# RoboticExplorationLab/TrajectoryOptimization.jl

Hardware: AMD Instinct MI355X
Metric: iLQR iterations/sec (batched trajectories) (higher is better)
Workload: dtype f64

## Files before the change

trajectoryoptimization.jl_amd/csrc/common.h:

```cpp
#pragma once
#include <hip/hip_runtime.h>

#include "models.h"
#include "problem_dev.h"

namespace to {

struct KArgs {
  DevProblem P;
  double* Xs;
  double* Us;
  double *Xc, *Uc;
  int dump_wave;
  int repack_block0;
  int CW, TW;
  double* x0;
  int* acc;
  int* accp;
  int coop_merge;
  int compact;
  int* alist;
  int* acount;
  int* ccount;
  double *Mc, *Hc, *gc;
  double* Kt;
  double *Mt, *Ht, *gt;
  int bwd_mfma;
  int bwd_lane;
  int h_compact;
  int h_diag;
  double *lam, *mu;
  double *J, *dJ, *grad, *rho, *drho, *dV, *cmax, *Jout;
  int *status, *iterations, *it_inner, *outer, *dJzero, *ls_index, *active, *budget, *bpfail;
  int* counter;
  int *oflag, *ost;
  int *olist, *ocount;
  double* knotbuf;
  double* mu_next;
  int* it_pn;
  double* pn_cmax;
  int al_mode;
  int control;
  int step;
  int ls_phase;
  int ls_c0;
  int blk0;
  int* pending;
  int* plist;
  int* pcount;
  int store_x;
};

struct PolicyArgs {
  int S;
  int TPW;
  int WPT;
  int g0;
  int store;
  int clamp;
  double alpha;
  double u_min[TO_MAX_M], u_max[TO_MAX_M];
  double mp[16];
  const double* x0s;
  double *J, *cmax, *dxmax;
  int *status, *klim;
  double *Xw, *Uw;
  const double* plants;
  double sigma_w[TO_MAX_N];
  double sigma_v[TO_MAX_N];
  unsigned long long seed;
  unsigned traj_offset, sample_offset;
};

template <class M> struct Gains { static constexpr int RSK = M::m * (M::ne + 1); };

#define TILE_PTR(base, L) ((base) + ((size_t)tile * (size_t)(L)) * 64 + lane)
#define EL(p, e) (p)[(size_t)(e) * 64]
#define TILE_LANE() const int tile = blockIdx.x, lane = threadIdx.x, b = tile * 64 + lane
__device__ __forceinline__ double* slot_ptr(double* nominal, double* cand, const int* accp, int b, int sl, int L) {
  if (sl == 0) return nominal + ((size_t)(b >> 6) * (size_t)L) * 64 + (b & 63);
  const int pos = accp[b];
  return cand + ((size_t)(pos >> 6) * (size_t)L) * 64 + (pos & 63);
}
#define X_SLOT_PTR(a, b, sl) slot_ptr((a).Xs, (a).Xc, (a).accp, b, sl, (a).P.N * (a).P.n)
#define U_SLOT_PTR(a, b, sl) slot_ptr((a).Us, (a).Uc, (a).accp, b, sl, ((a).P.N - 1) * (a).P.m)

template <class M, bool GEN = true, class D = std::nullptr_t>
__device__ __forceinline__ double knot_cost(const DevProblem& P, int k, const double* x, const double* u, const double* lam0,
                                            const double* mu0, bool with_al, const double* gl0 = nullptr, const double* cp0 = nullptr,
                                            const double* cl0 = nullptr, D dt0 = nullptr) {
  constexpr int n = M::n, m = M::m, nz = n + m;
  const int cidx = P.cost_index[k];
  double Jk = cost_eval<n, m, GEN>(P.costs[cidx], x, u);
  if constexpr (GEN) {
    if (P.gl) Jk += goal_lin_cost<n, m>(gl0, cidx, x, u);
  }
  if (P.opts.cost_dt_scaling && k < P.N - 1) Jk *= step_dt(P, k, dt0);
  if (with_al && P.n_cons > 0) {
    double z[nz];
#pragma unroll
    for (int i = 0; i < n; ++i) z[i] = x[i];
#pragma unroll
    for (int i = 0; i < m; ++i) z[n + i] = u[i];
// ... 157 lines not shown
```

trajectoryoptimization.jl_amd/csrc/handle.h:

```cpp
#pragma once
#include <hip/hip_runtime.h>

#include <atomic>
#include <condition_variable>
#include <cstdint>
#include <mutex>
#include <string>
#include <thread>
#include <type_traits>
#include <vector>

#include "common.h"
#include "path_plan.h"
#include "rp_plan.h"

namespace to {

int fail(int code, const std::string& msg);

#define HIPCHECK(expr)                                                                         \
  do {                                                                                         \
    hipError_t e_ = (expr);                                                                    \
    if (e_ != hipSuccess)                                                                      \
      return ::to::fail(TO_ERR_HIP, std::string(#expr) + ": " + hipGetErrorString(e_));        \
  } while (0)
#define TRY(expr) do { int r_ = (expr); if (r_ != TO_OK) return r_; } while (0)

constexpr int BLOCK = 64;

template <class... P, class... A>
inline void enqueue(void (*kernel)(P...), dim3 grid, dim3 block, size_t lds, hipStream_t stream, const A&... args) {
  hipLaunchKernelGGL(kernel, grid, block, lds, stream, args...);
}
inline int launched() {
  HIPCHECK(hipGetLastError());
  return TO_OK;
}
template <class... P, class... A>
inline int launch(void (*kernel)(P...), dim3 grid, dim3 block, size_t lds, hipStream_t stream, const A&... args) {
  enqueue(kernel, grid, block, lds, stream, args...);
  return launched();
}

struct ModelOps;

}

struct to_handle_s {
  int device = 0;
  hipStream_t stream = nullptr;
  int model_key = -1;
  const to::ModelOps* ops = nullptr;
  int R = 0, G = 0;
  to::KArgs a;
  std::vector<to_cost_desc> costs;
  std::vector<to::DevCon> cons;
  std::vector<double> dt;
  std::vector<int> cost_index;
  std::vector<double> step_table;
  std::vector<void*> allocs;
  double* stage = nullptr;
  size_t stage_bytes = 0;
  int* counter_host = nullptr;
  int counter_len = 0;
  to::PathTraits traits;
  to::PathPlan plan;
  int accept_chunks = 1;
  to_cost_desc* d_costs = nullptr;
  to::DevCon* d_cons = nullptr;
  double* d_dt = nullptr;
  int* d_cost_index = nullptr;
  int* d_crow = nullptr;
  std::vector<char> gl_set;
  double* d_gl = nullptr;
  double* d_pm = nullptr;
  std::vector<double> pm_host;
  bool pm_own = false;
  double* d_dtb = nullptr;
  std::vector<double> dtb_host;
  double* d_cp = nullptr;
  double* d_cl = nullptr;
  std::vector<int> cl_base;
  std::vector<std::vector<double>> cl_host;
  double* d_tmp = nullptr;
  double* d_tmp2 = nullptr;
  void* comm = nullptr;
  int comm_rank = 0, comm_size = 1;
  std::vector<int32_t> comm_counts;
  long long comm_offset = 0, comm_total = 0;
  bool comm_equal = true;
  double* pn_ws = nullptr;
  size_t pn_ws_bytes = 0;
  int* pn_pak = nullptr;
  long long* pn_koff = nullptr;
  int* pn_list = nullptr;
  int* pn_list_host = nullptr;
  int pn_tab_len = 0;
  int pn_cap = 0, pn_nbmax = 0;
  long long pn_per = 0;
  hipStream_t pn_stream = nullptr;
  hipEvent_t pn_ev[3] = {nullptr, nullptr, nullptr};
  int32_t *snap_status = nullptr, *snap_active = nullptr;
  double* snap_cmax = nullptr;
  int pn_early = 0;
  std::vector<char> pn_done_early;
  int pn_early_slots = 0;
  to_solver_opts pn_opts;
  double pn_early_ms = 0.0;
  struct RpArr { size_t off; int kind; int L; };
  std::vector<RpArr> rp_arr;
  std::vector<void*> rp_home, rp_work[2];
  int* rp_map[2] = {nullptr, nullptr};
  to::RpSized rp_sized[2];
  int rp_level = 0;
  int rp_B = 0, rp_Bp = 0;
  double *pol_x0s = nullptr, *pol_J = nullptr, *pol_cmax = nullptr, *pol_dxmax = nullptr;
  int *pol_status = nullptr, *pol_klim = nullptr;
  size_t pol_cap = 0;
  double *pol_xw = nullptr, *pol_uw = nullptr;
// ... 104 lines not shown
```

trajectoryoptimization.jl_amd/csrc/k_forward.h:

```cpp
#pragma once
#include <type_traits>

#include "common.h"
#include "ls_round.h"

#ifndef TO_FWD_WAVES
#define TO_FWD_WAVES 1
#endif
namespace to {

template <class M, bool WITHK>
struct FwdKnot {
  static constexpr int n = M::n, m = M::m, RSK = Gains<M>::RSK;
  double x[n], u[m], kd[WITHK ? RSK : 1];
  __device__ __forceinline__ void load(const double* pXk, const double* pUk, const double* pKk) {
#pragma unroll
    for (int i = 0; i < n; ++i) x[i] = EL(pXk, i);
#pragma unroll
    for (int j = 0; j < m; ++j) u[j] = EL(pUk, j);
    if constexpr (WITHK) {
#pragma unroll
      for (int i = 0; i < RSK; ++i) kd[i] = pKk[i];
    }
  }
};

template <class M>
__device__ __forceinline__ void stage_gains(const double* Kt, int b, int TW, int k, int N, double* kbuf, int hw) {
  constexpr int RSK = Gains<M>::RSK;
  static_assert(RSK % 2 == 0, "gains rows must be whole 16-byte pieces");
  constexpr int PCS = RSK / 2;
  typedef __attribute__((address_space(1))) const void* gptr_t;
  typedef __attribute__((address_space(3))) void* lptr_t;
  const int pieces = TW * PCS;
  for (int i0 = 0; i0 < pieces; i0 += 64) {
    const int gl = i0 + hw;
    int t = gl / PCS;
    const int off = gl - t * PCS;
    t = t < TW ? t : TW - 1;
    const int bt = __shfl(b, t);
    const char* src = (const char*)(Kt + ((size_t)bt * (N - 1) + k) * RSK) + off * 16;
    __builtin_amdgcn_global_load_lds((gptr_t)src, (lptr_t)((char*)kbuf + (size_t)i0 * 16), 16, 0, 0);
  }
}
template <class M>
__host__ __device__ inline int gains_lds_doubles(int TW) {
  constexpr int PCS = Gains<M>::RSK / 2;
  return ((TW * PCS + 63) / 64) * 64 * 2;
}

template <class M, int MODE>
__device__ __forceinline__ void forward_candidate(const KArgs& a, int tile, int lane, int b, bool live, double alpha, int wblock, double* kbuf,
                                                  int kbuf_len, int krow, int b0, int TW, int hw, double& J_out, double& g_out, bool& ok_out) {
  constexpr int n = M::n, m = M::m, ne = M::ne, RSK = Gains<M>::RSK;
  constexpr bool SIMPLE = (MODE & 1) != 0, CONS = (MODE & 2) != 0, GEN = (MODE & 8) != 0;
  constexpr bool KLDS = M::lds_gains;
// ... 634 lines not shown
        if (ncs > 0) Ja += cs0.term(ub);
        if (ncs > 1) Ja += cs1.term(ub);
        Jk += Ja;
      } else Jk += knot_al_cached<M, GEN>(P, k, xb, ub, lam0, mu0, ncs, cs0, cs1, cp0, cl0);
    }
    J += Jk;
    double mx = 0.0, mu_ = 0.0;
    if (k > 0) {
#pragma unroll
      for (int i = 0; i < n; ++i) { const double v = fabs(xb[i]); if (!(v <= mx)) mx = v; }
    }
#pragma unroll
    for (int j = 0; j < m; ++j) { const double v = fabs(ub[j]); if (!(v <= mu_)) mu_ = v; }
    if (!(mx <= max_x) || !(mu_ <= max_u)) ok = false;
  }
  FWD2_BARRIER();
  {
    double xb[n + 1];
    const double2* slot = (const double2*)(ring + (size_t)((N - 1) & 1) * R::SLOT) + hw;
#pragma unroll
    for (int pr = 0; pr < (n + 1) / 2; ++pr) { const double2 v = slot[pr * 64]; xb[2 * pr] = v.x; if (2 * pr + 1 < n + 1) xb[2 * pr + 1] = v.y; }
    double mx = 0.0;
#pragma unroll
    for (int i = 0; i < n; ++i) { const double v = fabs(xb[i]); if (!(v <= mx)) mx = v; }
    if (!(mx <= max_x)) ok = false;
#pragma unroll
    for (int i = 0; i < n; ++i) EL(pXo, i) = xb[i];
    double u0[m];
#pragma unroll
    for (int j = 0; j < m; ++j) u0[j] = 0.0;
    J += knot_cost<M, GEN>(P, N - 1, xb, u0, lam0, mu0, true, gl0, cp0, cl0);
  }
  J_out = J; g_out = gsum / (N - 1); ok_out = ok;
}

#ifndef TO_FWD2_WAVES
#define TO_FWD2_WAVES 1
#endif
template <class M>
__host__ __device__ inline size_t fwd2_lds_doubles(int TW) {
  return (M::lds_gains ? 2 * (size_t)gains_lds_doubles<M>(TW) + StageCostLds<M::n, M::m>::size : 0) + 2 * (size_t)Fwd2Ring<M>::SLOT + 2;
}
template <class M, int MODE>
__global__ void __launch_bounds__(128, TO_FWD2_WAVES) k_forward2(KArgs a) {
  extern __shared__ double kbuf[];
  const DevProblem& P = a.P;
  const to_solver_opts& o = P.opts;
  const int hw = threadIdx.x & 63;
  const int role = __builtin_amdgcn_readfirstlane(threadIdx.x >> 6);
  const int CW = a.CW, TW = a.TW;
  const int q = hw / TW, t = hw - q * TW;
  const int b0 = blockIdx.x * TW;
  int b, inrange;
  if (a.compact) {
    const int cnt = a.acount[a.step & 1];
    if (b0 >= cnt) return;
    inrange = (b0 + t) < cnt;
    b = a.alist[(size_t)(a.step & 1) * P.Bp + (inrange ? b0 + t : cnt - 1)];
  } else {
    inrange = (b0 + t) < P.B;
    b = (b0 + t) < P.Bp ? b0 + t : P.Bp - 1;
  }
  const int tile = b >> 6, lane = b & 63;
  const bool act = inrange && a.active[b] != 0;
  if (__ballot(act) == 0) return;
  const bool bpfail = act && a.bpfail[b] != 0;
  const int total = o.iterations_linesearch;
  const double Jprev = a.J[b];
  const double dV0 = a.dV[b], dV1 = a.dV[(size_t)P.Bp + b];
  const bool zero_step = act && !bpfail && (-(dV0 + dV1) <= 1e-12 * (1.0 + fabs(Jprev)));
  bool need = act && !bpfail && !zero_step;
  int accepted = zero_step ? 0 : -1, acc = 0, accpos = 0;
  double Jnew = Jprev, grad = 0.0;
  const double f = o.line_search_decrease_factor;
  const int kbuf_len = M::lds_gains ? gains_lds_doubles<M>(TW) : 0;
  const unsigned long long tmask = TW >= 64 ? ~0ull : (1ull << TW) - 1ull;
  double* ctab = kbuf + 2 * (size_t)kbuf_len;
  double* ring = ctab + (M::lds_gains ? StageCostLds<M::n, M::m>::size : 0);
  unsigned long long* needmask = (unsigned long long*)(ring + 2 * (size_t)Fwd2Ring<M>::SLOT);
  if constexpr (!LsRepack<M>::value) {
    const int krow = t * Gains<M>::RSK;
    unsigned long long nm = __ballot(need);
    for (int c0 = 0; c0 < total; c0 += CW) {
      if (nm == 0) break;
      const double alpha = ls_alpha(f, c0 + q, total);
      if (role == 0) {
        fwd2_roll<M, MODE>(a, tile, lane, b, alpha, kbuf, kbuf_len, krow, TW, hw, ring);
      } else {
        const bool cand = need && q < CW && (c0 + q) < total;
        double J, gm;
        bool ok;
        fwd2_account<M, MODE>(a, tile, lane, b, cand, (int)blockIdx.x, ctab, hw, ring, J, gm, ok);
        bool accept = false;
        if (cand && ok) {
          const double expected = -alpha * (dV0 + alpha * dV1);
          const double z = (expected > 0.0) ? (Jprev - J) / expected : -1.0;
          accept = z >= o.line_search_lower_bound && z <= o.line_search_upper_bound;
        }
        const unsigned long long am = __ballot(accept);
        int qs = -1;
        for (int qq = CW - 1; qq >= 0; --qq) qs = ((am >> (qq * TW + t)) & 1ull) ? qq : qs;
        const int src = (qs >= 0 ? qs : 0) * TW + t;
        const double Js = __shfl(J, src), gs = __shfl(gm, src);
        if (need && qs >= 0) { Jnew = Js; grad = gs; accepted = c0 + qs; acc = qs + 1; accpos = (int)blockIdx.x * 64 + src; need = false; }
        const unsigned long long left = __ballot(need);
        if (hw == 0) *needmask = left;
      }
// ... 53 lines not shown
```

trajectoryoptimization.jl_amd/csrc/k_misc.h:

```cpp
#pragma once
#include "common.h"

namespace to {

template <class M, int FIXED_INTEG, bool PM = false, bool DT = false>
__global__ void __launch_bounds__(64) k_rollout(KArgs a) {
  constexpr int n = M::n, m = M::m;
  TILE_LANE();
  const DevProblem& P = a.P;
  if (b >= P.B) return;
  constexpr int c = 0;
  double* X = X_SLOT_PTR(a, b, c);
  const double* U = U_SLOT_PTR(a, b, c);
  const double* x0 = TILE_PTR(a.x0, n);
  double x[n], u[m], xn[n];
  double pmr[PM ? 16 : 1];
  const double* mp = P.mp;
  if constexpr (PM) { load_plant(P, b, pmr); mp = pmr; }
  const double* dt0 = dt_lane_of<DT>(P, b);
#pragma unroll
  for (int i = 0; i < n; ++i) { x[i] = EL(x0, i); EL(X, i) = x[i]; }
  int lim = 0;
  const double max_x = P.opts.max_state_value, max_u = P.opts.max_control_value;
  for (int k = 0; k < P.N - 1; ++k) {
#pragma unroll
    for (int i = 0; i < m; ++i) u[i] = EL(U, k * m + i);
    model_step<M, double, FIXED_INTEG>(mp, P.integrator, k, x, u, step_dt_of<DT>(P, k, dt0), xn);
    double mx = 0.0, mu = 0.0;
#pragma unroll
    for (int i = 0; i < n; ++i) { x[i] = xn[i]; EL(X, (k + 1) * n + i) = x[i]; const double v = fabs(x[i]); mx = !(v <= mx) ? v : mx; }
#pragma unroll
    for (int i = 0; i < m; ++i) { const double v = fabs(u[i]); mu = !(v <= mu) ? v : mu; }
    if (lim == 0) lim = !(mx <= max_x) ? TO_STATE_LIMIT : !(mu <= max_u) ? TO_CONTROL_LIMIT : 0;
  }
  if (a.control && lim != 0 && a.active[b] != 0) {
    a.status[b] = lim; a.active[b] = 0;
    if (a.al_mode) a.outer[b] = 1;
  }
}

template <class M>
__global__ void __launch_bounds__(64) k_cost(KArgs a, int with_al, double* out, double* Jk) {
  constexpr int n = M::n, m = M::m;
  TILE_LANE();
  const DevProblem& P = a.P;
  if (b >= P.B) return;
  const int N = P.N;
  if (Jk) {
    constexpr int c = 0;
    const double* X = X_SLOT_PTR(a, b, c);
    const double* U = U_SLOT_PTR(a, b, c);
    double* o = TILE_PTR(Jk, N);
    const double* dt0 = dt_lane(P, b);
    for (int k = 0; k < N; ++k) {
      double x[n], u[m];
#pragma unroll
      for (int i = 0; i < n; ++i) x[i] = EL(X, k * n + i);
#pragma unroll
      for (int i = 0; i < m; ++i) u[i] = (k < N - 1) ? EL(U, k * m + i) : 0.0;
      EL(o, k) = knot_cost<M>(P, k, x, u, nullptr, nullptr, false, TILE_PTR(P.gl, P.n_costs * (n + m)), nullptr, nullptr, dt0);
    }
    return;
  }
  double J;
  trajectory_pass<M>(a, tile, lane, with_al != 0, false, &J, nullptr);
  out[b] = J;
}

template <class M>
__global__ void __launch_bounds__(64) k_violation(KArgs a, double* out) {
  TILE_LANE();
  if (b >= a.P.B) return;
  double cm;
  trajectory_pass<M>(a, tile, lane, false, false, nullptr, &cm);
  out[b] = cm;
}

template <class M>
__global__ void __launch_bounds__(64) k_dual_update(KArgs a) {
  TILE_LANE();
  const DevProblem& P = a.P;
  if (b >= P.B) return;
  trajectory_pass<M>(a, tile, lane, false, true, nullptr, nullptr);
  double* mu0 = TILE_PTR(a.mu, P.n_cons);
  for (int ci = 0; ci < P.n_cons; ++ci) EL(mu0, ci) = fmin(EL(mu0, ci) * P.opts.penalty_scaling, P.opts.penalty_max);
}


#define OUTER_LANE(FLAG)                                                                      \
  const DevProblem& P = a.P;                                                                  \
  const int cnt_ = a.ocount[a.step & 1];                                                      \
// ... 271 lines not shown
```

trajectoryoptimization.jl_amd/csrc/k_scan.h:

```cpp
#pragma once
#include "common.h"
#include "k_backward.h"
#include "k_expand.h"
#include "scan_combine.h"

namespace to {

__device__ __forceinline__ double scan_shfl(double v, int src_lane) {
  return __shfl(v, src_lane);
}

template <int n, bool VALUE_ONLY, bool SELECT>
__device__ __forceinline__ void scan_round(const ScanEl<n>& el, int l, int d, ScanEl<n>& out) {
  using E = ScanEl<n>;
  E pe;
  const int src = l + d;
  const bool has = src < 64;
  const int sl = has ? src : 63;
  if constexpr (VALUE_ONLY) {
#pragma unroll
    for (int i = 0; i < n; ++i) pe.eta[i] = scan_shfl(el.eta[i], sl);
#pragma unroll
    for (int i = 0; i < E::NSY; ++i) pe.J[i] = scan_shfl(el.J[i], sl);
    if constexpr (SELECT) {
      if (!has) {
#pragma unroll
        for (int i = 0; i < n; ++i) pe.eta[i] = 0.0;
#pragma unroll
        for (int i = 0; i < E::NSY; ++i) pe.J[i] = 0.0;
      }
    }
  } else {
    const double* pv = (const double*)&el;
    double* po = (double*)&pe;
#pragma unroll
    for (int i = 0; i < E::NV; ++i) po[i] = scan_shfl(pv[i], sl);
    if constexpr (SELECT) {
      if (!has) pe.identity();
    }
  }
  scan_combine<n, VALUE_ONLY>(el, pe, out);
}

template <class M>
__device__ __forceinline__ bool scan_element(const double* Mk, const double* Hd, const double* g, bool terminal, bool beyond,
                                             ScanEl<M::ne>& e) {
  constexpr int m = M::m, ne = M::ne, nc = ne + m;
  using E = ScanEl<ne>;
  bool ok = true;
  double iR[m];
#pragma unroll
  for (int c = 0; c < m; ++c) { if (!terminal && not_positive(Hd[ne + c])) ok = false; iR[c] = rcp_fast(terminal ? 1.0 : Hd[ne + c]); }
#pragma unroll
  for (int i = 0; i < ne; ++i) {
// ... 142 lines not shown
#pragma unroll
    for (int i = 0; i < ne; ++i) {
      double t = Qxx[i][j];
#pragma unroll
      for (int r = 0; r < m; ++r) t += Kg[r][i] * W[r][j];
#pragma unroll
      for (int r = 0; r < m; ++r) t += Qux[r][i] * Kg[r][j];
      Sn[i][j] = t;
    }
    double t = gq[j];
#pragma unroll
    for (int r = 0; r < m; ++r) t += Kg[r][j] * qd[r];
#pragma unroll
    for (int r = 0; r < m; ++r) t += Qux[r][j] * dk[r];
    sn[j] = t;
  }
  double dv1 = 0.0, dv2 = 0.0;
#pragma unroll
  for (int r = 0; r < m; ++r) {
    dv1 += dk[r] * gq[ne + r];
    double t = 0.0;
#pragma unroll
    for (int q = 0; q < m; ++q) t += Quu[r][q] * dk[q];
    dv2 += dk[r] * t;
  }
  dv1o = dv1; dv2o = 0.5 * dv2;
#pragma unroll
  for (int i = 0; i < ne; ++i) {
#pragma unroll
    for (int j = 0; j < ne; ++j) S[i][j] = 0.5 * (Sn[i][j] + Sn[j][i]);
    s[i] = sn[i];
  }
  return pd_ok;
}

#ifndef TO_SCAN_PRIO
#define TO_SCAN_PRIO 1
#endif
template <class M, int FIXED_INTEG, int VAR, bool TRIM = true>
__global__ void __launch_bounds__(64, 1) k_expand_backward_scan(KArgs a) {
  static_assert(!M::lie && M::ne <= 4 && M::m <= 2, "scan backward pass: small vector-space models");
  constexpr int n = M::n, m = M::m, ne = M::ne, nc = ne + m, RSK = Gains<M>::RSK;
  constexpr int PK = ne * nc + 2 * nc;
  using E = ScanEl<ne>;
  using LL = LaneLay<M>;
  __shared__ double park[2 * PK * 64];
#if TO_SCAN_PRIO
  if constexpr (TRIM) __builtin_amdgcn_s_setprio(TO_SCAN_PRIO);
#endif
  const DevProblem& P = a.P;
  const int N = P.N;
  const int b = blockIdx.x, l = threadIdx.x;
  const int tile = b >> 6, lane = b & 63;
  double rho = a.rho[b], drho = a.drho[b];
  if (!a.active[b]) return;
  const int c = M::accept_write_through ? a.acc[b] : 0;
  const double* X = X_SLOT_PTR(a, b, c);
  const double* U = U_SLOT_PTR(a, b, c);
  double* X0 = X_SLOT_PTR(a, b, 0);
  double* U0 = U_SLOT_PTR(a, b, 0);
  const bool wt = M::accept_write_through && c != 0;
  bool ok = true;
  E el;
  {
    E e0, e1;
#pragma unroll
    for (int kk = 0; kk < 2; ++kk) {
      const int kr = 2 * l + kk;
      const bool beyond = kr > N - 1;
      const int k = beyond ? N - 1 : kr;
      const bool terminal = (k == N - 1);
      double x[n], u[m];
#pragma unroll
      for (int i = 0; i < n; ++i) x[i] = EL(X, k * n + i);
#pragma unroll
      for (int i = 0; i < m; ++i) u[i] = terminal ? 0.0 : EL(U, k * m + i);
      if (wt && !beyond) {
#pragma unroll
        for (int i = 0; i < n; ++i) EL(X0, k * n + i) = x[i];
        if (!terminal) {
#pragma unroll
          for (int i = 0; i < m; ++i) EL(U0, k * m + i) = u[i];
        }
      }
      double Mk[ne * nc], H[LL::NS], g[nc], Hd[nc];
#pragma unroll
      for (int i = 0; i < ne * nc; ++i) Mk[i] = 0.0;
      expand_lane_knot<M, FIXED_INTEG, VAR>(a, tile, lane, k, x, u, Mk, H, g, a.P.mp);
#pragma unroll
      for (int j = 0; j < nc; ++j) { Hd[j] = (terminal && j >= ne) ? 1.0 : H[LL::sym(j, j)]; if (terminal && j >= ne) g[j] = 0.0; }
      double* pk = park + (size_t)kk * PK * 64 + l;
#pragma unroll
      for (int i = 0; i < ne * nc; ++i) pk[i * 64] = Mk[i];
#pragma unroll
      for (int j = 0; j < nc; ++j) { pk[(ne * nc + j) * 64] = Hd[j]; pk[(ne * nc + nc + j) * 64] = g[j]; }
      const bool eok = scan_element<M>(Mk, Hd, g, terminal, beyond, kk == 0 ? e0 : e1);
      if (!eok && !beyond) ok = false;
    }
    scan_combine<ne>(e0, e1, el);
  }
  double dV0 = 0.0, dV1 = 0.0;
  double* pK = a.Kt + ((size_t)b * (N - 1)) * RSK;
  bool done = false, failed = false;
  const bool elements_ok = __ballot(!ok) == 0;
  if (rho == 0.0 && elements_ok) {
    const int NB = (N + 1) / 2;
    int d = 1;
  #pragma unroll 1
    for (; (TRIM ? 2 * d : d) < NB; d <<= 1) {
      E out;
      scan_round<ne, false, !TRIM>(el, l, d, out);
      el = out;
    }
    if constexpr (TRIM) {
      if (d < NB) {
        E out;
        scan_round<ne, true, false>(el, l, d, out);
  #pragma unroll
        for (int i = 0; i < ne; ++i) el.eta[i] = out.eta[i];
  #pragma unroll
        for (int i = 0; i < E::NSY; ++i) el.J[i] = out.J[i];
      }
    }
    double S[ne][ne], s[ne];
    {
      const int src = (l + 1 < 64) ? l + 1 : 63;
      double Jn[E::NSY], en[ne];
  #pragma unroll
      for (int i = 0; i < E::NSY; ++i) Jn[i] = scan_shfl(el.J[i], src);
// ... 97 lines not shown
```

trajectoryoptimization.jl_amd/csrc/ops.h:

```cpp
#pragma once
#include <cstdlib>
#include <type_traits>

#include "handle.h"
#include "k_backward.h"
#include "k_expand.h"
#include "k_forward.h"
#include "k_scan.h"
#include "k_misc.h"
#include "k_policy.h"

namespace to {

template <class M>
void fill_traits(ModelOps& o) {
  o.write_through = M::accept_write_through;
  o.mfma_backward = M::mfma_backward;
  o.coop_backward = M::coop_backward;
  o.lane_backward = M::lane_backward;
  o.lds_gains = M::lds_gains;
  o.expand_knots = M::expand_knots;
  o.ls_first_round = M::ls_first_round;
  o.gains_lds_pieces = Gains<M>::RSK / 2;
  if constexpr (M::mfma_backward) {
// ... 161 lines not shown
  return fail(TO_ERR_UNSUPPORTED, "fused expansion + cooperative backward pass not compiled for this model");
}

template <class M>
int op_expand_backward_scan(to_handle* h) {
  if constexpr (!M::lie && M::ne <= 4 && M::m <= 2) {
    const DevProblem& P = h->a.P;
    if (P.expand_variant != 0 || !h->a.h_diag || P.N > 126) return fail(TO_ERR_UNSUPPORTED, "scan backward pass: outside its scope");
    const char* env = std::getenv("TRAJOPT_SCAN_TRIM");
    const bool trim = !(env && std::atoi(env) == 0);
    return with_integrator<M>(h, [&](auto fi) {
      constexpr int FI = decltype(fi)::value;
      if (!trim) return launch(k_expand_backward_scan<M, FI, 0, false>, dim3(P.B), dim3(64), 0, h->stream, h->a);
      return launch(k_expand_backward_scan<M, FI, 0, true>, dim3(P.B), dim3(64), 0, h->stream, h->a);
    });
  }
  return fail(TO_ERR_UNSUPPORTED, "scan backward pass not compiled for this model");
}

template <class M, int MODE>
int op_forward(to_handle* h) {
  const KArgs& a = h->a;
  const int TW = a.TW;
  const size_t lds = M::lds_gains ? sizeof(double) * (2 * gains_lds_doubles<M>(TW) + StageCostLds<M::n, M::m>::size) : 0;
  return with_time_steps<M, (MODE & 32) != 0>(h, [&](auto dt) {
    return launch(k_forward<M, (MODE | (decltype(dt)::value ? 64 : 0))>, dim3((a.P.Bp + TW - 1) / TW), dim3(BLOCK), lds, h->stream, a);
  });
}

template <class M>
int op_accept_roll(to_handle* h) {
  enqueue(k_accept_gather_u<M>, grid_b(h), dim3(BLOCK), 0, h->stream, h->a);
  return with_integrator<M>(h, [&](auto fi) { return launch(k_accept_roll<M, decltype(fi)::value>, grid_b(h), dim3(BLOCK), 0, h->stream, h->a); });
}

template <class M, int NZ = 0>
int op_policy_rollout(to_handle* h, const PolicyArgs& pa, int waves) {
  const bool uniform = pa.TPW == 0;
  const size_t lds = M::lds_gains ? sizeof(double) * 2 * gains_lds_doubles<M>(uniform ? 1 : pa.TPW) : 0;
  return with_integrator<M>(h, [&](auto fi) {
    return with_time_steps<M, (NZ & 4) != 0>(h, [&](auto dt) {
      constexpr int FI = decltype(fi)::value;
      constexpr bool DT = decltype(dt)::value;
      if (uniform) return launch(k_policy_rollout<M, true, FI, NZ, DT>, dim3(waves), dim3(BLOCK), lds, h->stream, h->a, pa);
      return launch(k_policy_rollout<M, false, FI, NZ, DT>, dim3(waves), dim3(BLOCK), lds, h->stream, h->a, pa);
    });
  });
}

template <class M, int MODE>
int op_forward2(to_handle* h) {
  const KArgs& a = h->a;
  const int TW = a.TW;
  return launch(k_forward2<M, MODE>, dim3((a.P.Bp + TW - 1) / TW), dim3(128), sizeof(double) * fwd2_lds_doubles<M>(TW), h->stream, a);
}
template <class M, int LO, int HI>
void fill_forward2(ModelOps& o) {
  if constexpr (LO < HI) {
    if constexpr (M::pin_rk4 || (LO & 4) == 0) o.forward2[LO] = op_forward2<M, LO>;
    fill_forward2<M, LO + 1, HI>(o);
  }
}
template <class M, int GEN>
void fill_forward_pm(ModelOps& o) {
  static_assert((GEN & 8) != 0 && GEN < 32, "per-trajectory model parameters: general forward variants only");
  if constexpr (M::pin_rk4 || (GEN & 4) == 0) o.forward[1][GEN] = op_forward<M, (GEN | 32)>;
}

template <class M>
void fill_misc(ModelOps& o) {
  fill_traits<M>(o);
  o.rollout[0] = op_rollout<M>; o.cost = op_cost<M>; o.violation = op_violation<M>; o.dual_update = op_dual_update<M>;
  o.outer = op_outer<M>; o.cost_derivs = op_cost_derivs<M>; o.discrete_jacobian[0] = op_discrete_jacobian<M>;
  o.constraint_eval = op_constraint_eval<M>; o.constraint_hessian = op_constraint_hessian<M>;
}
template <class M, int LO, int HI>
void fill_forward(ModelOps& o) {
  if constexpr (LO < HI) {
    if constexpr (M::pin_rk4 || (LO & 4) == 0) o.forward[0][LO] = op_forward<M, LO>;
    fill_forward<M, LO + 1, HI>(o);
  }
}

}
```

trajectoryoptimization.jl_amd/csrc/path_plan.h:

```cpp
#pragma once

#include <algorithm>
#include <cstdint>
#include <cstdlib>
#include <cstring>

namespace to {

struct PathTraits {
  bool write_through = false, mfma_backward = false, coop_backward = true, lane_backward = false;
  int ls_first_round = 16;
  bool expand_backward = false, expand_backward_coop = false, expand_backward_scan = false, accept_roll = false, expand_lane_k = false, expand_const = false;
  uint32_t forward = 0, forward2 = 0;
  uint32_t forward_plants = 0;
};
struct PathShape {
  int B = 1, Bp = 64, N = 2, ne = 1, m = 1, n_cons = 0, iterations_linesearch = 20;
  bool diagonal_cost_blocks = false;
  int cus = 256;
};
struct PathKnobs {
  int ls_candidates = 0, ls_deep = 1, scan = 1, backward = 0, expand_lane = 1, fused_coop = 1, fused_lane = 1, accept_roll_min = -1, repack = 16384,
      expand_pack = 1, fwd2 = 2, coop_merge = 1, scan_max = 1 << 30, ls_repack = 1, ls_two_a = 2, ls_two_b = 2, compact = 1;
  double accept_roll_frac = 0.25, repack_at = 0.7;
// ... 68 lines not shown
  if (k.backward == 2 && t.mfma_backward) { p.bwd_mfma = 1; p.bwd_lane = 0; }
  if (k.backward == 3 && t.lane_backward) { p.bwd_mfma = 0; p.bwd_lane = 1; }
  p.fused_coop = (!p.bwd_lane && !p.bwd_mfma && t.expand_backward_coop && k.fused_coop) ? 1 : 0;
  p.expand_lane = k.expand_lane; p.expand_pack = k.expand_pack; p.fwd2 = k.fwd2; p.coop_merge = k.coop_merge; p.scan_max_active = k.scan_max;
  p.roll_min_active = k.accept_roll_min; p.roll_min_frac = k.accept_roll_frac; p.rp_min = k.repack; p.rp_at = k.repack_at;
  p.scan = (p.fused_coop && t.expand_backward_scan && s.N <= 126 && k.scan) ? (k.scan == 2 ? 2 : 1) : 0;
  p.fused_lane = (p.bwd_lane && t.expand_backward && k.fused_lane) ? 1 : 0;
  p.compact = ((p.fused_lane || p.bwd_mfma) && k.compact) ? 1 : 0;
  p.waves = wave_blocks(Bp, p.tw_base);
  if (p.cw_deep) p.waves = std::max(p.waves, wave_blocks(Bp, p.tw_deep));
  p.dump_wave = (int)p.waves;
  long long extra = 0;
  if (!t.write_through && k.ls_repack) { extra = p.waves; p.repack_block0 = (int)p.waves + 1; }
  p.x_blocks = p.u_blocks = p.waves + 1 + extra;
  if (t.write_through && t.accept_roll && Bp >= 32768) {
    const int ca = k.ls_two_a, cb = k.ls_two_b;
    if (ca >= 1 && ca <= 16 && cb >= 1 && cb <= 16 && ca < s.iterations_linesearch) {
      const long long nA = wave_blocks(Bp, 64 / ca), nB = wave_blocks(Bp, 64 / cb);
      p.ls2_cwa = ca; p.ls2_cwb = cb; p.ls2_blkA = (int)nA; p.ls2_dump = (int)(nA + nB);
      p.u_blocks = std::max(p.u_blocks, nA + nB + 1);
    }
  }
  return p;
}
inline bool fused_coop_now(const PathPlan& p, int h_diag, int expand_variant, bool plants = false) {
  return !plants && p.fused_coop && h_diag && (expand_variant == 0 || expand_variant == 2);
}
inline bool scan_now(const PathPlan& p, int h_diag, int expand_variant, bool plants = false) {
  return p.scan && fused_coop_now(p, h_diag, expand_variant, plants) && expand_variant == 0;
}
inline int solve_compact(const PathPlan& p, bool plants = false) { return (plants && !p.bwd_mfma) ? 0 : p.compact; }
inline int roll_min(const PathPlan& p, const PathTraits& t) { return p.roll_min_active >= 0 ? p.roll_min_active : t.write_through ? 32768 : 2048; }
inline bool working_set_repack(const PathPlan& p, const PathTraits& t, bool plants = false) {
  return !plants && p.fused_lane && p.compact && t.write_through && p.rp_min > 0;
}
enum StepKind { STEP_SPLIT, STEP_FUSED_LANE, STEP_FUSED_COOP, STEP_SCAN };
struct StepPlan { StepKind kind; int CW, TW; bool two_wave; int store_x; bool two_launch; };
inline StepPlan plan_step(const PathPlan& p, const PathTraits& t, int h_diag, int expand_variant, int compact_armed, int last_active, int B,
                          bool plants = false) {
  StepPlan s;
  s.kind = (p.fused_lane && !plants) ? STEP_FUSED_LANE
           : scan_now(p, h_diag, expand_variant, plants) && last_active <= p.scan_max_active ? STEP_SCAN
           : fused_coop_now(p, h_diag, expand_variant, plants) ? STEP_FUSED_COOP
           : STEP_SPLIT;
  const bool deep = p.cw_deep && last_active <= p.deep_max_active;
  s.CW = deep ? p.cw_deep : p.cw_base; s.TW = deep ? p.tw_deep : p.tw_base;
  s.two_wave = !plants && p.fwd2 == 2 && 2 * wave_blocks(last_active, s.TW) <= (long long)p.simds;
  const int rmin = roll_min(p, t);
  const bool dense = !t.write_through || (double)last_active >= p.roll_min_frac * (double)B;
  s.store_x = (!plants && rmin > 0 && t.accept_roll && !s.two_wave && last_active >= rmin && dense) ? 0 : 1;
  s.two_launch = !s.store_x && p.ls2_cwa && compact_armed && p.fwd2 != 1;
  return s;
}
inline void path_report(const PathPlan& p, const PathTraits& t, int h_diag, int expand_variant, int B, int32_t info[8], bool plants = false) {
  info[0] = p.bwd_mfma ? 1 : p.bwd_lane ? 2 : 0;
  info[1] = ((p.fused_lane && !plants) || fused_coop_now(p, h_diag, expand_variant, plants)) ? 1 : 0;
  info[2] = solve_compact(p, plants);
  info[3] = p.cw_base;
  info[4] = (!plants && p.fwd2 && t.forward2) ? 2 : 1;
  info[5] = scan_now(p, h_diag, expand_variant, plants) ? 1 : 0;
  info[6] = (!plants && t.accept_roll && p.roll_min_active != 0) ? 1 : 0;
  info[7] = p.repack_block0 != 0 ? 1 : 0;
  if (working_set_repack(p, t, plants) && B >= p.rp_min) info[7] |= 2;
}
struct TableFlags {
  bool dense_costs = false, cons = false, non_selector = false;
  bool con_params = false, con_limits = false, plants = false;
  bool time_steps = false;
};
inline bool routed_as_plants(bool plants , bool time_steps ) { return plants || time_steps; }
inline bool routed_as_plants(const TableFlags& f) { return routed_as_plants(f.plants, f.time_steps); }
inline int expand_variant_of(const TableFlags& f) {
  return (f.dense_costs ? 1 : 0) | (f.cons ? 2 : 0) | ((f.non_selector || f.con_params || f.con_limits || routed_as_plants(f)) ? 4 : 0);
}
inline bool forward_general(int expand_variant, bool cost_terms , bool con_params , bool con_limits ) {
  return (expand_variant & 5) != 0 || cost_terms || con_params || con_limits;
}
inline int forward_mode(bool simple_stage, bool has_cons, bool rk4, bool general, bool unit_soc, uint32_t mask) {
  auto has = [&](int mode) { return (mask >> mode) & 1u; };
  int mode = (simple_stage ? 1 : 0) | (has_cons ? 2 : 0) | (rk4 ? 4 : 0) | (general ? 8 : 0);
  if (!has(mode)) mode &= ~4;
  if (unit_soc && has(mode | 16)) mode |= 16;
  if (!has(mode)) mode = (mode | 8) & ~1 & ~16;
  return has(mode) ? mode : -1;
}
constexpr int COMPACT_ONE_LAUNCH = 16384;
inline bool compact_grid(int Bp, int* per, int* nb) {
  *per = std::min(65536, ((Bp + 255) / 256 + 1023) / 1024 * 1024);
  *nb = (Bp + *per - 1) / *per;
  return *nb <= 256;
}

}
```

trajectoryoptimization.jl_amd/csrc/trajopt_hip.hip:

```cpp
#include <hip/hip_runtime.h>

#include <algorithm>
#include <cmath>
#include <cstdio>
#include <cstdlib>
#include <cstring>
#include <string>
#include <vector>

#include <dlfcn.h>
#include <time.h>

#include <mutex>
#include <thread>

#include "desc_lower.h"
#include "handle.h"
#include "k_generic.h"
#include "k_mpc.h"

using namespace to;

namespace {
thread_local std::string g_err;
}
namespace to {
int fail(int code, const std::string& msg) { g_err = msg; return code; }
}

namespace to {
constexpr size_t GUARD_BYTES = 4096;
constexpr unsigned long long GUARD_WORD = 0xA5C3A5C3DEADBEEFull;
struct GuardZones { unsigned long long* front; unsigned long long* back; };
__global__ void k_guard_fill(unsigned long long* z) { z[blockIdx.x * 64 + threadIdx.x] = GUARD_WORD; }
__global__ void k_guard_check(const GuardZones* tab, int* bad) {
  const GuardZones g = tab[blockIdx.x];
  constexpr int words = (int)(GUARD_BYTES / 8);
  bool hit = false;
  for (int i = threadIdx.x; i < words; i += 64) hit = hit || g.front[i] != GUARD_WORD || g.back[i] != GUARD_WORD;
  if (hit) atomicMin(bad, (int)blockIdx.x);
}
__global__ void k_guard_poke(double* p, long long off) { p[off] = 1.0; }

int g_malloc(to_handle* h, void** p, size_t bytes, const char* name) {
  if (!h->guard) {
    HIPCHECK(hipMalloc(p, bytes));
    return TO_OK;
  }
  const size_t payload = (bytes + 255) / 256 * 256;
  void* base = nullptr;
  HIPCHECK(hipMalloc(&base, payload + 2 * GUARD_BYTES));
  char* q = (char*)base + GUARD_BYTES;
  enqueue(k_guard_fill, dim3(GUARD_BYTES / 8 / 64), dim3(64), 0, h->stream, (unsigned long long*)base);
  enqueue(k_guard_fill, dim3(GUARD_BYTES / 8 / 64), dim3(64), 0, h->stream, (unsigned long long*)(q + payload));
  if (payload > bytes) HIPCHECK(hipMemsetAsync(q + bytes, 0, payload - bytes, h->stream));
  TRY(launched());
  h->guards.push_back({base, q, payload, name ? name : ""});
  h->guard_dirty = true;
  *p = q;
  return TO_OK;
}
void g_free(to_handle* h, void* p) {
  if (!p) return;
  if (h->guard)
    for (size_t i = 0; i < h->guards.size(); ++i)
      if (h->guards[i].payload == p) {
        hipFree(h->guards[i].base);
        h->guards.erase(h->guards.begin() + i);
        h->guard_dirty = true;
// ... 341 lines not shown
  dbg_sync("k_repack_home");
  TRY(launch(k_repack_move, dim3((count + 63) / 64, mv.n), dim3(64), 0, h->stream, mv, list, count, omap_old, h->rp_map[w]));
  dbg_sync("k_repack_move");
  for (int i = 0; i < mv.n; ++i) rp_field(h, h->rp_arr[i].off) = h->rp_work[w][i];
  a.P.B = count; a.P.Bp = Bp_new;
  TRY(launch(k_repack_list, dim3((count + 255) / 256), dim3(256), 0, h->stream, a.alist + (size_t)next * a.P.Bp, a.acount + next, count));
  h->rp_level = lvl + 1;
  return TO_OK;
}
int rp_finish(to_handle* h, bool copy) {
  if (h->rp_level == 0) return TO_OK;
  KArgs& a = h->a;
  const int w = (h->rp_level - 1) & 1;
  int rc = TO_OK;
  if (copy) {
    RpArgs hm;
    hm.n = (int)h->rp_arr.size();
    for (int i = 0; i < hm.n; ++i) { hm.kind[i] = h->rp_arr[i].kind; hm.L[i] = h->rp_arr[i].L; hm.src[i] = rp_field(h, h->rp_arr[i].off); hm.dst[i] = h->rp_home[i]; }
    if (launch(k_repack_home, dim3((a.P.B + 63) / 64, hm.n), dim3(64), 0, h->stream, hm, a.active, a.P.B, h->rp_map[w], 1) != TO_OK)
      rc = fail(TO_ERR_HIP, "k_repack_home launch failed");
  }
  for (size_t i = 0; i < h->rp_arr.size(); ++i) rp_field(h, h->rp_arr[i].off) = h->rp_home[i];
  a.P.B = h->rp_B; a.P.Bp = h->rp_Bp;
  h->rp_level = 0;
  return rc;
}

void trace_line(to_handle* h, int active, int steps, const char* tag) {
  static const char* path = std::getenv("TRAJOPT_TRACE");
  if (!path) return;
  static std::mutex mu;
  static FILE* f = std::fopen(path, "a");
  if (!f) return;
  timespec ts;
  clock_gettime(CLOCK_MONOTONIC, &ts);
  std::lock_guard<std::mutex> lk(mu);
  std::fprintf(f, "%p %.6f %d %d %s\n", (void*)h, ts.tv_sec + 1e-9 * ts.tv_nsec, steps, active, tag);
  std::fflush(f);
}
void publish_progress(to_handle* h, int active, int steps) {
  trace_line(h, active, steps, "step");
  const int before = h->prog_active.exchange(active);
  h->prog_steps = steps;
  if (active < before) { std::lock_guard<std::mutex> lk(h->prog_mu); h->prog_cv.notify_all(); }
}
int solve_impl(to_handle* h, to_solve_stats* st, int al_mode);
int solve(to_handle* h, to_solve_stats* st, int al_mode) {
  int rc = solve_impl(h, st, al_mode);
  if (rc == TO_OK && h->guard) rc = check_guards(h, "the end of a solve (final accept, working set home, statistics)");
  publish_progress(h, 0, h->prog_steps);
  rp_finish(h, false);
  h->a.control = 0;
  h->a.compact = 0;
  h->a.CW = h->plan.cw_base; h->a.TW = h->plan.tw_base;
  h->a.store_x = 1;
  return rc;
}
int pn_run(to_handle* h, const std::vector<int>& list, const to_solver_opts& opts) {
  if (list.empty()) return TO_OK;
  if (!h->ops->pn_launch[0]) return fail(TO_ERR_UNSUPPORTED, "projected Newton not compiled for this model");
  const int count = (int)list.size();
  TRY(h->ops->pn_prepare(h, count));
  hipEvent_t e0 = h->sev[0], e1 = h->sev[1];
  HIPCHECK(hipEventRecord(e0, h->stream));
  std::memcpy(h->pn_list_host, list.data(), sizeof(int) * count);
  for (int base = 0; base < count; base += h->pn_cap) {
    const int cnt = std::min(h->pn_cap, count - base);
    HIPCHECK(hipMemcpyAsync(h->pn_list, h->pn_list_host + base, sizeof(int) * cnt, hipMemcpyHostToDevice, h->stream));
    TRY(launch_pn(h, 0, cnt, h->stream, &opts));
  }
  HIPCHECK(hipEventRecord(e1, h->stream));
  HIPCHECK(hipEventSynchronize(e1));
  float ms = 0.f;
  HIPCHECK(hipEventElapsedTime(&ms, e0, e1));
  h->last_ms += ms;
  if (h->profile) { h->prof_ms[3] += ms; h->prof_launches[3] += 1; }
  if (h->guard) TRY(check_guards(h, "the projected-Newton polish"));
  return TO_OK;
}
int ensure_solve_events(to_handle* h) {
  if (!h->sev[0]) {
    HIPCHECK(hipEventCreate(&h->sev[0]));
    HIPCHECK(hipEventCreate(&h->sev[1]));
    HIPCHECK(hipEventCreateWithFlags(&h->sev[2], hipEventDisableTiming));
    HIPCHECK(hipEventCreateWithFlags(&h->sev[3], hipEventDisableTiming));
  }
  return TO_OK;
}

int early_polish_setup(to_handle* h) {
  if (!h->pn_stream) {
    int lo = 0, hi = 0;
    HIPCHECK(hipDeviceGetStreamPriorityRange(&lo, &hi));
    HIPCHECK(hipStreamCreateWithPriority(&h->pn_stream, hipStreamNonBlocking, lo));
    HIPCHECK(hipEventCreateWithFlags(&h->pn_ev[0], hipEventDisableTiming));
    HIPCHECK(hipEventCreate(&h->pn_ev[1]));
    HIPCHECK(hipEventCreate(&h->pn_ev[2]));
    const size_t Bp = h->a.P.Bp;
    HIPCHECK(hipHostMalloc((void**)&h->snap_status, sizeof(int32_t) * Bp));
    HIPCHECK(hipHostMalloc((void**)&h->snap_active, sizeof(int32_t) * Bp));
    HIPCHECK(hipHostMalloc((void**)&h->snap_cmax, sizeof(double) * Bp));
  }
  return TO_OK;
}
int early_polish_snapshot(to_handle* h) {
  const KArgs& a = h->a;
// ... 47 lines not shown
  if (const char* env = std::getenv("TRAJOPT_PN_EARLY")) early = std::max(0, std::min(8, std::atoi(env)));
  h->pn_early = 0; h->pn_early_slots = 0;
  if (early > 0 && h->ops->pn_launch[0] && !h->ops->write_through) {
    if (h->ops->pn_prepare(h, B) == TO_OK && h->pn_cap >= B) {
      TRY(early_polish_setup(h));
      h->pn_done_early.assign(B, 0);
      h->pn_opts = user;
      h->pn_early = early;
    }
  }
  const bool had_early = h->pn_early > 0;
  h->a.P.opts.constraint_tolerance = user.projected_newton_tolerance;
  const int rc = solve(h, nullptr, 1);
  h->a.P.opts = user;
  h->pn_early = 0;
  if (had_early && h->pn_early_slots > 0) {
    const hipError_t e = hipEventSynchronize(h->pn_ev[1]);
    if (rc == TO_OK) HIPCHECK(e);
  }
  if (rc != TO_OK) return rc;
  if (had_early && h->pn_early_slots > 0) {
    float ms = 0.f, tail = 0.f;
    HIPCHECK(hipEventElapsedTime(&ms, h->pn_ev[2], h->pn_ev[1]));
    if (h->profile) { h->prof_ms[3] += ms; h->prof_launches[3] += 1; }
    HIPCHECK(hipEventElapsedTime(&tail, h->sev[1], h->pn_ev[1]));
    if (tail > 0.f) h->last_ms += tail;
  }
  std::vector<int32_t> status(B);
  std::vector<double> cmax(B);
  TRY(download_int(h, status.data(), h->a.status));
  TRY(download_scalar(h, cmax.data(), h->a.cmax));
  std::vector<int> list;
  for (int b = 0; b < B; ++b)
    if (status[b] == TO_SOLVE_SUCCEEDED && cmax[b] > user.constraint_tolerance && !(had_early && h->pn_done_early[b])) list.push_back(b);
  trace_line(h, (int)list.size(), h->last_steps, "polish");
  const int prc = pn_run(h, list, user);
  trace_line(h, 0, h->last_steps, "polish_done");
  if (prc != TO_OK && prc != TO_ERR_UNSUPPORTED) return prc;
  if (st) { const std::string note = prc == TO_OK ? std::string() : g_err; TRY(fill_stats(h, st, true)); if (!note.empty()) g_err = "polish skipped: " + note; }
  return TO_OK;
}

int solve_impl(to_handle* h, to_solve_stats* st, int al_mode) {
  TRY(use_device(h));
  KArgs& a = h->a;
  const DevProblem& P = a.P;
  a.al_mode = al_mode;
  a.control = 1;
  h->rp_arr.clear();
  a.compact = solve_compact(h->plan, plants(h) != 0);
  const int max_steps = (al_mode ? P.opts.iterations_total : P.opts.iterations) + 1;
  if (h->counter_len < max_steps) {
    int* c = nullptr;
    TRY(g_malloc(h, (void**)&c, sizeof(int) * max_steps, "step counters"));
    h->allocs.push_back(c);
    a.counter = c;
    if (h->counter_host) HIPCHECK(hipHostFree(h->counter_host));
    HIPCHECK(hipHostMalloc((void**)&h->counter_host, sizeof(int) * max_steps));
    h->counter_len = max_steps;
  }
  HIPCHECK(hipMemsetAsync(a.counter, 0, sizeof(int) * max_steps, h->stream));
  TRY(ensure_solve_events(h));
  const hipEvent_t e0 = h->sev[0], e1 = h->sev[1];
  HIPCHECK(hipEventRecord(e0, h->stream));
  HIPCHECK(hipMemsetAsync(a.it_pn, 0, sizeof(int) * P.Bp, h->stream));
  TRY(launch(k_solve_init, grid_b(h), dim3(BLOCK), 0, h->stream, a, al_mode));
  TRY(launch_rollout(h));
  TRY(launch_cost(h, 1, a.J, nullptr));
  if (a.compact) {
    a.step = -1;
    TRY(launch_compact(h));
  }
  int steps = 0;
  if (h->profile) {
    while ((int)h->ev.size() < 4 * max_steps) { hipEvent_t e; HIPCHECK(hipEventCreate(&e)); h->ev.push_back(e); }
  }
  constexpr int CHECK_EVERY = 4;
  const hipEvent_t cev[2] = {h->sev[2], h->sev[3]};
  int launched = 0, checked = 0, nchunks = 0, last_active = P.B;
  bool done = false;
  h->prog_active = P.B; h->prog_steps = 0;
  const bool dbg_sync = std::getenv("TRAJOPT_SYNC_DEBUG") != nullptr;
  auto enqueue_chunk = [&]() -> int {
    const int chunk = std::min(CHECK_EVERY, max_steps - launched);
    for (int c = 0; c < chunk; ++c) {
      const int step = launched + c;
      a.step = step;
      if (h->profile) HIPCHECK(hipEventRecord(h->ev[4 * step + 0], h->stream));
      const PathPlan& pl = h->plan;
      const StepPlan sp = plan_step(pl, h->traits, a.h_diag, P.expand_variant, a.compact, last_active, P.B, plants(h) != 0);
      if (sp.kind == STEP_SPLIT) TRY(launch_expand(h));
      if (h->profile) HIPCHECK(hipEventRecord(h->ev[4 * step + 1], h->stream));
      switch (sp.kind) {
        case STEP_FUSED_LANE: TRY(h->ops->expand_backward(h)); break;
        case STEP_SCAN: TRY(h->ops->expand_backward_scan(h)); break;
        case STEP_FUSED_COOP: TRY(h->ops->expand_backward_coop(h)); break;
        case STEP_SPLIT: TRY(launch_backward(h)); break;
      }
      if (h->profile) HIPCHECK(hipEventRecord(h->ev[4 * step + 2], h->stream));
      a.CW = sp.CW; a.TW = sp.TW; a.store_x = sp.store_x;
      if (sp.two_launch) {
        const int cw0 = a.CW, tw0 = a.TW, dump0 = a.dump_wave;
        a.dump_wave = pl.ls2_dump;
        a.CW = pl.ls2_cwa; a.TW = 64 / pl.ls2_cwa; a.ls_phase = 1; a.blk0 = 0;
        TRY(launch_forward(h, false, false));
        TRY(launch_flag_list(h));
        a.CW = pl.ls2_cwb; a.TW = 64 / pl.ls2_cwb; a.ls_phase = 2; a.ls_c0 = pl.ls2_cwa; a.blk0 = pl.ls2_blkA;
        TRY(launch_forward(h, false, false));
        a.ls_phase = 0; a.blk0 = 0; a.CW = cw0; a.TW = tw0; a.dump_wave = dump0;
        TRY(launch_accept(h));
      } else
      TRY(launch_forward(h, !h->ops->write_through || !a.store_x, sp.two_wave));
      a.store_x = 1;
      if (al_mode) TRY(launch_outer(h));
      if (a.compact) TRY(launch_compact(h));
      if (h->profile) HIPCHECK(hipEventRecord(h->ev[4 * step + 3], h->stream));
      if (h->guard) {
        if (step == 0) if (const char* env = std::getenv("TRAJOPT_GUARD_SELFTEST")) if (std::atoi(env))
          enqueue(k_guard_poke, dim3(1), dim3(1), 0, h->stream, a.Xs, (long long)P.N * P.n * (P.Bp + 64) + 3);
        TRY(check_guards(h, ("batch step " + std::to_string(step) + " of a solve").c_str()));
      }
      if (dbg_sync) {
        const hipError_t e = hipStreamSynchronize(h->stream);
        std::fprintf(stderr, "[sync-debug] step %d B=%d Bp=%d level=%d store_x-path=%d: %s\n", step, a.P.B, a.P.Bp, h->rp_level, (int)(last_active), hipGetErrorString(e));
        if (e != hipSuccess) return fail(TO_ERR_HIP, "device fault (sync debug)");
      }
    }
    HIPCHECK(hipMemcpyAsync(&h->counter_host[launched], &a.counter[launched], sizeof(int) * chunk, hipMemcpyDeviceToHost, h->stream));
    HIPCHECK(hipEventRecord(cev[nchunks & 1], h->stream));
    launched += chunk;
    ++nchunks;
    return TO_OK;
  };
  int waited = 0;
  int early_div = 4;
  if (const char* env = std::getenv("TRAJOPT_PN_EARLY_AT")) early_div = std::max(1, std::atoi(env));
  int early_thr = (al_mode && h->pn_early > 0) ? P.B / early_div : -1, early_left = h->pn_early;
  bool snapshot_pending = false;
  bool repack = !al_mode && a.compact && working_set_repack(h->plan, h->traits, plants(h) != 0);
  if (max_steps > 0) TRY(enqueue_chunk());
  while (!done && waited < nchunks) {
    if (repack && last_active >= 1 && (double)last_active <= h->plan.rp_at * (double)a.P.B && a.P.B >= h->plan.rp_min) {
      HIPCHECK(hipStreamSynchronize(h->stream));
      for (; checked < launched; ++checked) {
        ++steps;
        last_active = h->counter_host[checked];
        if (last_active == 0) { done = true; break; }
      }
      waited = nchunks;
      publish_progress(h, last_active, steps);
      if (done) break;
      a.step = launched - 1;
      {
// ... 1492 lines not shown
```

Baseline: 10.49 million.

## Build active-trajectory list in scan backward to shrink forward2 launch grid

The fused scan backward kernel now computes each active trajectory's rank with wave ballots over the active flags and writes its index into a double-buffered list. The forward2 line-search kernel reads trajectory ids from that list and launches only enough groups for the last known active count. Inactive trajectories with a pending accepted candidate copy it back to the nominal buffers. The aim is to stop launching forward work for converged trajectories without a separate compaction pass. The cost is an extra ballot/popcount pass per trajectory in backward and a per-step active count kept in a counter slot just before the step counters.

```diff
diff --git a/trajectoryoptimization.jl_amd/csrc/common.h b/trajectoryoptimization.jl_amd/csrc/common.h
--- a/trajectoryoptimization.jl_amd/csrc/common.h
+++ b/trajectoryoptimization.jl_amd/csrc/common.h
@@ -49,6 +49,7 @@
   int* plist;
   int* pcount;
   int store_x;
+  int fwd_list;
 };
 
 struct PolicyArgs {
diff --git a/trajectoryoptimization.jl_amd/csrc/fwd_list.h b/trajectoryoptimization.jl_amd/csrc/fwd_list.h
--- /dev/null
+++ b/trajectoryoptimization.jl_amd/csrc/fwd_list.h
@@ -0,0 +1,17 @@
+#pragma once
+
+namespace to {
+
+constexpr int FWD_LIST_MAX_BP = 2048;
+constexpr int FWD_LIST_CHUNK = 16;
+
+__host__ __device__ __forceinline__ int fwd_list_passes(int b) { return (b + 63) >> 6; }
+__host__ __device__ __forceinline__ int fwd_list_rank_add(unsigned long long mask, int p, int b) {
+  const int d = b - 64 * p, below = d < 0 ? 0 : d;
+  const unsigned long long keep = below >= 64 ? ~0ull : (1ull << below) - 1ull;
+  return __builtin_popcountll(mask & keep);
+}
+__host__ __device__ __forceinline__ long long fwd_list_slot(int step, int Bp, int rank) { return (long long)(step & 1) * Bp + rank; }
+__host__ __device__ __forceinline__ int fwd_list_groups(int count, int TW) { return count < 1 ? 1 : (count + TW - 1) / TW; }
+
+}
diff --git a/trajectoryoptimization.jl_amd/csrc/handle.h b/trajectoryoptimization.jl_amd/csrc/handle.h
--- a/trajectoryoptimization.jl_amd/csrc/handle.h
+++ b/trajectoryoptimization.jl_amd/csrc/handle.h
@@ -65,6 +65,7 @@
   int counter_len = 0;
   to::PathTraits traits;
   to::PathPlan plan;
+  int list_active = 0;
   int accept_chunks = 1;
   to_cost_desc* d_costs = nullptr;
   to::DevCon* d_cons = nullptr;
diff --git a/trajectoryoptimization.jl_amd/csrc/k_forward.h b/trajectoryoptimization.jl_amd/csrc/k_forward.h
--- a/trajectoryoptimization.jl_amd/csrc/k_forward.h
+++ b/trajectoryoptimization.jl_amd/csrc/k_forward.h
@@ -2,6 +2,7 @@
 #include <type_traits>
 
 #include "common.h"
+#include "fwd_list.h"
 #include "ls_round.h"
 
 #ifndef TO_FWD_WAVES
@@ -742,7 +743,14 @@
   const int q = hw / TW, t = hw - q * TW;
   const int b0 = blockIdx.x * TW;
   int b, inrange;
-  if (a.compact) {
+  if (a.fwd_list) {
+    const int pos = b0 + t < P.Bp ? b0 + t : P.Bp - 1;
+    const int entry = a.alist[fwd_list_slot(a.step, P.Bp, pos)];
+    const int cnt = a.counter[a.step - 1];
+    if (b0 >= cnt) return;
+    inrange = (b0 + t) < cnt;
+    b = inrange ? entry : __builtin_amdgcn_readfirstlane(entry);
+  } else if (a.compact) {
     const int cnt = a.acount[a.step & 1];
     if (b0 >= cnt) return;
     inrange = (b0 + t) < cnt;
diff --git a/trajectoryoptimization.jl_amd/csrc/k_misc.h b/trajectoryoptimization.jl_amd/csrc/k_misc.h
--- a/trajectoryoptimization.jl_amd/csrc/k_misc.h
+++ b/trajectoryoptimization.jl_amd/csrc/k_misc.h
@@ -37,6 +37,7 @@
     a.status[b] = lim; a.active[b] = 0;
     if (a.al_mode) a.outer[b] = 1;
   }
+  if (a.fwd_list && a.control && a.active[b] != 0) atomicAdd(&a.counter[-1], 1);
 }
 
 template <class M>
diff --git a/trajectoryoptimization.jl_amd/csrc/k_scan.h b/trajectoryoptimization.jl_amd/csrc/k_scan.h
--- a/trajectoryoptimization.jl_amd/csrc/k_scan.h
+++ b/trajectoryoptimization.jl_amd/csrc/k_scan.h
@@ -1,5 +1,6 @@
 #pragma once
 #include "common.h"
+#include "fwd_list.h"
 #include "k_backward.h"
 #include "k_expand.h"
 #include "scan_combine.h"
@@ -248,8 +249,32 @@
   const int N = P.N;
   const int b = blockIdx.x, l = threadIdx.x;
   const int tile = b >> 6, lane = b & 63;
+  const int act = a.active[b];
+  const bool listed = a.fwd_list != 0;
+  const int np = listed ? fwd_list_passes(b) : 0;
+  long long lslot = fwd_list_slot(a.step, P.Bp, 0);
+  asm volatile("" : "+s"(lslot));
+  int f0[FWD_LIST_CHUNK];
+  if (np > 0) {
+#pragma unroll
+    for (int i = 0; i < FWD_LIST_CHUNK; ++i) f0[i] = a.active[(size_t)(i < np ? i : np - 1) * 64 + l];
+  }
   double rho = a.rho[b], drho = a.drho[b];
-  if (!a.active[b]) return;
+  if (!act) {
+    if constexpr (M::accept_write_through) {
+      if (listed && a.acc[b] != 0) {
+        const int Lx = N * n, Lu = (N - 1) * m;
+        const double* cx = X_SLOT_PTR(a, b, 1);
+        const double* cu = U_SLOT_PTR(a, b, 1);
+        double* nx = X_SLOT_PTR(a, b, 0);
+        double* nu = U_SLOT_PTR(a, b, 0);
+        for (int e = l; e < Lx; e += 64) EL(nx, e) = EL(cx, e);
+        for (int e = l; e < Lu; e += 64) EL(nu, e) = EL(cu, e);
+        if (l == 0) a.acc[b] = 0;
+      }
+    }
+    return;
+  }
   const int c = M::accept_write_through ? a.acc[b] : 0;
   const double* X = X_SLOT_PTR(a, b, c);
   const double* U = U_SLOT_PTR(a, b, c);
@@ -271,6 +296,23 @@
       for (int i = 0; i < n; ++i) x[i] = EL(X, k * n + i);
 #pragma unroll
       for (int i = 0; i < m; ++i) u[i] = terminal ? 0.0 : EL(U, k * m + i);
+      if (kk == 0 && listed) {
+        int rank = 0;
+        if (np > 0) {
+#pragma unroll
+          for (int i = 0; i < FWD_LIST_CHUNK; ++i) asm volatile("" : "+v"(f0[i]));
+#pragma unroll
+          for (int i = 0; i < FWD_LIST_CHUNK; ++i) rank += fwd_list_rank_add(__ballot(f0[i] != 0), i, b);
+        }
+        for (int p0 = FWD_LIST_CHUNK; p0 < np; p0 += FWD_LIST_CHUNK) {
+          int f[FWD_LIST_CHUNK];
+#pragma unroll
+          for (int i = 0; i < FWD_LIST_CHUNK; ++i) f[i] = a.active[(size_t)(p0 + i < np ? p0 + i : np - 1) * 64 + l];
+#pragma unroll
+          for (int i = 0; i < FWD_LIST_CHUNK; ++i) rank += fwd_list_rank_add(__ballot(f[i] != 0), p0 + i, b);
+        }
+        if (l == 0) a.alist[lslot + rank] = b;
+      }
       if (wt && !beyond) {
 #pragma unroll
         for (int i = 0; i < n; ++i) EL(X0, k * n + i) = x[i];
diff --git a/trajectoryoptimization.jl_amd/csrc/ops.h b/trajectoryoptimization.jl_amd/csrc/ops.h
--- a/trajectoryoptimization.jl_amd/csrc/ops.h
+++ b/trajectoryoptimization.jl_amd/csrc/ops.h
@@ -237,7 +237,8 @@
 int op_forward2(to_handle* h) {
   const KArgs& a = h->a;
   const int TW = a.TW;
-  return launch(k_forward2<M, MODE>, dim3((a.P.Bp + TW - 1) / TW), dim3(128), sizeof(double) * fwd2_lds_doubles<M>(TW), h->stream, a);
+  const int groups = a.fwd_list ? fwd_list_groups(h->list_active, TW) : (a.P.Bp + TW - 1) / TW;
+  return launch(k_forward2<M, MODE>, dim3(groups), dim3(128), sizeof(double) * fwd2_lds_doubles<M>(TW), h->stream, a);
 }
 template <class M, int LO, int HI>
 void fill_forward2(ModelOps& o) {
diff --git a/trajectoryoptimization.jl_amd/csrc/path_plan.h b/trajectoryoptimization.jl_amd/csrc/path_plan.h
--- a/trajectoryoptimization.jl_amd/csrc/path_plan.h
+++ b/trajectoryoptimization.jl_amd/csrc/path_plan.h
@@ -144,6 +144,13 @@
   s.two_launch = !s.store_x && p.ls2_cwa && compact_armed && p.fwd2 != 1;
   return s;
 }
+inline bool solve_forward_list(const PathPlan& p, const PathTraits& t, int h_diag, int expand_variant, int compact_armed, int al_mode, int B, int Bp,
+                               bool plants, bool linear_terms, bool forward2_compiled, bool enabled, int max_bp) {
+  if (!enabled || al_mode || compact_armed || plants || linear_terms || !forward2_compiled || !t.write_through || Bp > max_bp) return false;
+  const StepPlan full = plan_step(p, t, h_diag, expand_variant, compact_armed, B, B, plants);
+  if (full.kind != STEP_SCAN || !full.store_x || full.two_launch) return false;
+  return full.two_wave || p.fwd2 == 1;
+}
 inline void path_report(const PathPlan& p, const PathTraits& t, int h_diag, int expand_variant, int B, int32_t info[8], bool plants = false) {
   info[0] = p.bwd_mfma ? 1 : p.bwd_lane ? 2 : 0;
   info[1] = ((p.fused_lane && !plants) || fused_coop_now(p, h_diag, expand_variant, plants)) ? 1 : 0;
diff --git a/trajectoryoptimization.jl_amd/csrc/trajopt_hip.hip b/trajectoryoptimization.jl_amd/csrc/trajopt_hip.hip
--- a/trajectoryoptimization.jl_amd/csrc/trajopt_hip.hip
+++ b/trajectoryoptimization.jl_amd/csrc/trajopt_hip.hip
@@ -15,6 +15,7 @@
 #include <thread>
 
 #include "desc_lower.h"
+#include "fwd_list.h"
 #include "handle.h"
 #include "k_generic.h"
 #include "k_mpc.h"
@@ -462,6 +463,7 @@
   rp_finish(h, false);
   h->a.control = 0;
   h->a.compact = 0;
+  h->a.fwd_list = 0;
   h->a.CW = h->plan.cw_base; h->a.TW = h->plan.tw_base;
   h->a.store_x = 1;
   return rc;
@@ -615,14 +617,22 @@
   const int max_steps = (al_mode ? P.opts.iterations_total : P.opts.iterations) + 1;
   if (h->counter_len < max_steps) {
     int* c = nullptr;
-    TRY(g_malloc(h, (void**)&c, sizeof(int) * max_steps, "step counters"));
+    TRY(g_malloc(h, (void**)&c, sizeof(int) * (max_steps + 1), "step counters"));
     h->allocs.push_back(c);
-    a.counter = c;
+    a.counter = c + 1;
     if (h->counter_host) HIPCHECK(hipHostFree(h->counter_host));
     HIPCHECK(hipHostMalloc((void**)&h->counter_host, sizeof(int) * max_steps));
     h->counter_len = max_steps;
   }
-  HIPCHECK(hipMemsetAsync(a.counter, 0, sizeof(int) * max_steps, h->stream));
+  HIPCHECK(hipMemsetAsync(a.counter - 1, 0, sizeof(int) * (max_steps + 1), h->stream));
+  {
+    const char* env = std::getenv("TRAJOPT_FWD_LIST");
+    const int mode = forward_mode(P.simple_stage, P.n_cons > 0, P.integrator == INTEG_RK4,
+                                  forward_general(P.expand_variant, P.gl != nullptr, P.cp != nullptr, P.cl != nullptr), P.unit_soc, h->traits.forward);
+    a.fwd_list = solve_forward_list(h->plan, h->traits, a.h_diag, P.expand_variant, a.compact, al_mode, P.B, P.Bp, plants(h) != 0, P.gl != nullptr,
+                                    mode >= 0 && h->ops->forward2[mode] != nullptr && h->ops->expand_backward_scan != nullptr,
+                                    !(env && std::atoi(env) == 0), FWD_LIST_MAX_BP) ? 1 : 0;
+  }
   TRY(ensure_solve_events(h));
   const hipEvent_t e0 = h->sev[0], e1 = h->sev[1];
   HIPCHECK(hipEventRecord(e0, h->stream));
@@ -662,6 +672,7 @@
       }
       if (h->profile) HIPCHECK(hipEventRecord(h->ev[4 * step + 2], h->stream));
       a.CW = sp.CW; a.TW = sp.TW; a.store_x = sp.store_x;
+      h->list_active = last_active;
       if (sp.two_launch) {
         const int cw0 = a.CW, tw0 = a.TW, dump0 = a.dump_wave;
         a.dump_wave = pl.ls2_dump;
```

After: 11.17 million (median of 6 runs). 1.06x the previous value.
